# prj-beatrice/beatrice-vst

Measured on AMD Instinct MI355X. Metric: audio frames/sec (24 kHz out, 10 ms hop), higher is better.
Workload: dtype f32

## Files before the change

### beatrice-vst_amd/csrc/ring.h

```cpp
#pragma once
#include <hip/hip_runtime.h>

struct Ring {
  float* base;
  int C;
  int n;
  int m;
};

template <class T>
__device__ __forceinline__ T* as_global(T* p) {
  const unsigned long long v = reinterpret_cast<unsigned long long>(p);
  const unsigned long long u = (unsigned long long)(unsigned)__builtin_amdgcn_readfirstlane((int)(unsigned)v) |
                               ((unsigned long long)(unsigned)__builtin_amdgcn_readfirstlane((int)(unsigned)(v >> 32)) << 32);
  __attribute__((address_space(1))) T* g = (__attribute__((address_space(1))) T*)reinterpret_cast<T*>(u);
  asm("" : "+s"(g));
  return (T*)g;
}
template <class T>
__device__ __forceinline__ T* as_global_v(T* p) {
  __attribute__((address_space(1))) T* g = (__attribute__((address_space(1))) T*)p;
  asm("" : "+v"(g));
  return (T*)g;
}
__device__ __forceinline__ void globalize(Ring& r) { r.base = as_global(r.base); }

__host__ __device__ inline int ring_frames(const Ring& r) { return r.n * r.m; }
__host__ __device__ inline size_t ring_stream_floats(const Ring& r) { return (size_t)r.n * r.m * r.C; }

__device__ __forceinline__ int ring_pos(const Ring& r, int hop) { return (hop % r.m) * r.n; }

__device__ __forceinline__ float* ring_frame(const Ring& r, int b, int pos, int rel) {
  int f = pos + rel;
  const int R = r.n * r.m;
  if (f < 0) f += R;
  return r.base + (unsigned)(b * R + f) * (unsigned)r.C;
}

namespace stepc {
__shared__ int pair[2];
__shared__ const int* hopv;
constexpr unsigned long long kImmediateTop = 1ull << 36;
constexpr int kImmediateMaxSlot = 4095;
constexpr unsigned kImmediateHopMask = 0xffffffu;
__host__ __device__ inline const int* immediate(int hop, int slot = 0) {
  return reinterpret_cast<const int*>(static_cast<unsigned long long>((unsigned)(hop + 2)) | (static_cast<unsigned long long>((unsigned)slot) << 24));
}
__device__ __forceinline__ int step(const int* p) {
  const unsigned long long v = reinterpret_cast<unsigned long long>(p);
  return v == 0 ? pair[0] : (v < kImmediateTop ? (int)((unsigned)v & kImmediateHopMask) - 2 : *p);
}
__device__ __forceinline__ int of(const int* p, const int hop, const int b) {
  if (reinterpret_cast<unsigned long long>(p) != 0) return hop;
  const int* v = hopv;
  return v != nullptr ? v[b] : hop;
}
__device__ __forceinline__ bool ragged(const int* p) { return reinterpret_cast<unsigned long long>(p) == 0 && hopv != nullptr; }
template <bool RAG> __device__ __forceinline__ int of_t(const int hop, const int b) {
  if constexpr (RAG) { const int* v = hopv; return v != nullptr ? v[b] : hop; }
  else return hop;
}
template <bool RAG> __device__ __forceinline__ bool rag_t() {
  if constexpr (RAG) return hopv != nullptr;
  else return false;
}
__device__ __forceinline__ int slot(const int* p) {
  const unsigned long long v = reinterpret_cast<unsigned long long>(p);
  return v == 0 ? pair[1] : (v < kImmediateTop ? (int)(v >> 24) : p[1]);
}
template <class A> __device__ __forceinline__ auto set_hop(A& a, const int* p, int) -> decltype((void)(a.hop = p)) { a.hop = p; }
template <class A> __device__ __forceinline__ auto set_hop(A& a, const int* p, long) -> decltype((void)(a.a.hop = p)) { a.a.hop = p; }
template <class A> __device__ __forceinline__ void set_hop(A&, const int*, ...) {}
}
```

### beatrice-vst_amd/csrc/rowchain.hip.h

```cpp
#pragma once
#include "meas_env.h"
#include <hip/hip_runtime.h>

#include <cstdlib>

#include "conv_gemm.hip.h"
#include "kernels_misc.hip.h"
#include "ring.h"
#include "spec_math.hip.h"

#ifdef ABL_WEIGHTS_HOT
#define ABL_KB(x) ((x) & 1)
#else
#define ABL_KB(x) (x)
#endif

#ifdef RC_TIMING
__device__ unsigned long long* g_rc_stamps;
#define RC_STAMP(i) do { if (threadIdx.x == 0) g_rc_stamps[(size_t)blockIdx.x * 16 + (i)] = __builtin_readcyclecounter(); } while (0)
#else
#define RC_STAMP(i) do { } while (0)
#endif

namespace rc {

constexpr int NTHR = 512, NWAVE = 8;
#ifndef RC_KPERM
#define RC_KPERM 1
#endif
constexpr bool KPERM = RC_KPERM != 0;
constexpr int AS = B_HID + (KPERM ? 8 : 2);
constexpr int TILE = 16 * AS;
constexpr int SS = B_KV_LEN + (KPERM ? 8 : 2);
constexpr int STILE = 16 * SS;
__host__ __device__ constexpr int kpos(int k) { return KPERM ? ((k & ~15) | ((k & 3) << 2) | ((k >> 2) & 3)) : k; }
constexpr int KSTEP = KPERM ? 4 : 1;
#ifndef RC_WMAP
#define RC_WMAP RC_KPERM
#endif
template <int ROWGROUPS >
__device__ __forceinline__ void piece_of(const int W, const int ln, int* r, int* q) {
  if constexpr (RC_WMAP != 0) { *r = 4 * (W % ROWGROUPS) + (ln >> 4); *q = 16 * (W / ROWGROUPS) + (ln & 15); }
  else { *r = W; *q = ln; }
}
__device__ __forceinline__ int lane_koff(const int lane) { return KPERM ? 4 * (lane >> 4) : (lane >> 4); }
__device__ __forceinline__ float4 lds_kblock(const float* __restrict__ p, const int kb) {
  if constexpr (KPERM) return *reinterpret_cast<const float4*>(p + kb * 16);
  else { const float* q = p + kb * 16; return make_float4(q[0], q[4], q[8], q[12]); }
}
__device__ __forceinline__ void store_perm4(float* __restrict__ row, const int n0, const float v0, const float v1, const float v2, const float v3) {
  if constexpr (KPERM) {
    float* d = row + kpos(n0);
    d[0] = v0; d[4] = v1; d[8] = v2; d[12] = v3;
  } else {
    float2* d = reinterpret_cast<float2*>(row + n0);
    d[0] = make_float2(v0, v1); d[1] = make_float2(v2, v3);
  }
}

#ifndef RC_PIN_PIPELINE
#define RC_PIN_PIPELINE 1
#endif
__device__ __forceinline__ void pin_pipeline() {
#if RC_PIN_PIPELINE
  asm volatile("" ::: "memory");
  __builtin_amdgcn_sched_barrier(0);
#endif
}
#ifndef RC_PREFETCH
#define RC_PREFETCH 8
#endif
template <int RT, int CG> __host__ __device__ constexpr int seg_depth() { return RT == 1 ? (CG <= 2 ? RC_PREFETCH : (CG <= 3 ? 4 : 2)) : (RT * CG <= 2 ? 8 : 4); }
template <int RT, int CG> struct SegHead { float4 v[seg_depth<RT, CG>()][CG]; };
template <int RT, int CG>
__device__ __forceinline__ void seg_head_load(SegHead<RT, CG>& h, const float4* const (&wf)[CG]) {
#pragma unroll
  for (int d = 0; d < seg_depth<RT, CG>(); ++d)
#pragma unroll
    for (int c = 0; c < CG; ++c) h.v[d][c] = wf[c][(size_t)d * 64];
}
template <int CG, int KB, bool HEAD = false>
__device__ __forceinline__ void mma_segment_p(f32x4 (&acc)[CG], const float* __restrict__ a, const float4* const (&wf)[CG], const SegHead<1, CG>* head = nullptr) {
  constexpr int D = seg_depth<1, CG>();
  static_assert(KB % D == 0, "segment length");
  float4 bq[D][CG];
  pin_pipeline();
#pragma unroll
  for (int d = 0; d < D; ++d)
#pragma unroll
    for (int c = 0; c < CG; ++c) { if constexpr (HEAD) bq[d][c] = head->v[d][c]; else bq[d][c] = wf[c][(size_t)d * 64]; }
  float4 an = lds_kblock(a, 0);
#pragma unroll
  for (int kb = 0; kb < KB; kb += D) {
#pragma unroll
    for (int d = 0; d < D; ++d) {
      float4 cur[CG];
#pragma unroll
      for (int c = 0; c < CG; ++c) cur[c] = bq[d][c];
      const float4 x = an;
      if (kb + d + D < KB) {
#pragma unroll
        for (int c = 0; c < CG; ++c) bq[d][c] = wf[c][(size_t)ABL_KB(kb + d + D) * 64];
      }
      if (kb + d + 1 < KB) an = lds_kblock(a, kb + d + 1);
      pin_pipeline();
#pragma unroll
      for (int c = 0; c < CG; ++c) acc[c] = __builtin_amdgcn_mfma_f32_16x16x4f32(cur[c].x, x.x, acc[c], 0, 0, 0);
#pragma unroll
      for (int c = 0; c < CG; ++c) acc[c] = __builtin_amdgcn_mfma_f32_16x16x4f32(cur[c].y, x.y, acc[c], 0, 0, 0);
#pragma unroll
      for (int c = 0; c < CG; ++c) acc[c] = __builtin_amdgcn_mfma_f32_16x16x4f32(cur[c].z, x.z, acc[c], 0, 0, 0);
#pragma unroll
      for (int c = 0; c < CG; ++c) acc[c] = __builtin_amdgcn_mfma_f32_16x16x4f32(cur[c].w, x.w, acc[c], 0, 0, 0);
    }
  }
}
template <int RT, int CG, int KB, bool HEAD = false>
__device__ __forceinline__ void mma_segment_rt(f32x4 (&acc)[RT][CG], const float* __restrict__ a, const int a_tile_stride,
                                               const float4* const (&wf)[CG], const SegHead<RT, CG>* head = nullptr) {
  constexpr int D = seg_depth<RT, CG>();
  static_assert(KB % D == 0, "segment length");
  float4 bq[D][CG];
  pin_pipeline();
#pragma unroll
  for (int d = 0; d < D; ++d)
#pragma unroll
    for (int c = 0; c < CG; ++c) { if constexpr (HEAD) bq[d][c] = head->v[d][c]; else bq[d][c] = wf[c][(size_t)d * 64]; }
  float4 an[RT];
#pragma unroll
  for (int t = 0; t < RT; ++t) an[t] = lds_kblock(a + t * a_tile_stride, 0);
#pragma unroll
  for (int kb = 0; kb < KB; kb += D) {
#pragma unroll
    for (int d = 0; d < D; ++d) {
      float4 cur[CG];
#pragma unroll
      for (int c = 0; c < CG; ++c) cur[c] = bq[d][c];
      float4 av[RT];
#pragma unroll
      for (int t = 0; t < RT; ++t) av[t] = an[t];
      if (kb + d + D < KB) {
#pragma unroll
        for (int c = 0; c < CG; ++c) bq[d][c] = wf[c][(size_t)ABL_KB(kb + d + D) * 64];
      }
      if (kb + d + 1 < KB) {
#pragma unroll
        for (int t = 0; t < RT; ++t) an[t] = lds_kblock(a + t * a_tile_stride, kb + d + 1);
      }
      pin_pipeline();
#pragma unroll
      for (int t = 0; t < RT; ++t)
#pragma unroll
        for (int c = 0; c < CG; ++c) acc[t][c] = __builtin_amdgcn_mfma_f32_16x16x4f32(cur[c].x, av[t].x, acc[t][c], 0, 0, 0);
#pragma unroll
      for (int t = 0; t < RT; ++t)
#pragma unroll
        for (int c = 0; c < CG; ++c) acc[t][c] = __builtin_amdgcn_mfma_f32_16x16x4f32(cur[c].y, av[t].y, acc[t][c], 0, 0, 0);
#pragma unroll
      for (int t = 0; t < RT; ++t)
#pragma unroll
        for (int c = 0; c < CG; ++c) acc[t][c] = __builtin_amdgcn_mfma_f32_16x16x4f32(cur[c].z, av[t].z, acc[t][c], 0, 0, 0);
#pragma unroll
      for (int t = 0; t < RT; ++t)
#pragma unroll
        for (int c = 0; c < CG; ++c) acc[t][c] = __builtin_amdgcn_mfma_f32_16x16x4f32(cur[c].w, av[t].w, acc[t][c], 0, 0, 0);
    }
  }
}
template <int CG, int KB>
__device__ __forceinline__ void mma_segment(f32x4 (&acc)[CG], const float* __restrict__ a, const float4* __restrict__ wf,
                                            const size_t tile_stride) {
  const float4* wfc[CG];
#pragma unroll
  for (int c = 0; c < CG; ++c) wfc[c] = wf + c * tile_stride;
  mma_segment_p<CG, KB>(acc, a, wfc);
}

template <int NSEG, int CG, class Epi4>
__device__ __forceinline__ void layer256(const float* const (&seg)[NSEG], const int as, const float* __restrict__ w_packed,
                                         const int wave, const int lane, Epi4 epi4) {
  constexpr int K = NSEG * 256;
  const float4* wf = reinterpret_cast<const float4*>(w_packed) + (size_t)wave * (K / 16) * 64 + lane;
  const size_t tile_stride = (size_t)NWAVE * (K / 16) * 64;
  f32x4 tot[CG];
#pragma unroll
  for (int s = 0; s < NSEG; ++s) {
    f32x4 acc[CG];
#pragma unroll
    for (int c = 0; c < CG; ++c) acc[c] = f32x4{0.f, 0.f, 0.f, 0.f};
    mma_segment<CG, 16>(acc, seg[s] + (lane & 15) * as + lane_koff(lane), wf + (size_t)s * 16 * 64, tile_stride);
#pragma unroll
    for (int c = 0; c < CG; ++c) {
      if (s == 0) tot[c] = acc[c];
      else { tot[c][0] = tot[c][0] + acc[c][0]; tot[c][1] = tot[c][1] + acc[c][1]; tot[c][2] = tot[c][2] + acc[c][2]; tot[c][3] = tot[c][3] + acc[c][3]; }
    }
  }
#pragma unroll
  for (int c = 0; c < CG; ++c) epi4(lane & 15, (wave + NWAVE * c) * 16 + (lane >> 4) * 4, tot[c]);
}

template <int HOPS = 1>
__device__ __forceinline__ void load_tile(float* __restrict__ dst, const Ring& ring, const int* sid , const int pos, const int rel,
                                          const int tid, const int* rowhop = nullptr) {
#pragma unroll
  for (int i = 0; i < 2; ++i) {
    const int idx = tid + i * NTHR;
    int r, q;
    piece_of<4>(idx >> 6, idx & 63, &r, &q);
    const int b = sid[r];
    float4 v = make_float4(0.f, 0.f, 0.f, 0.f);
    if (b >= 0) v = *reinterpret_cast<const float4*>(ring_frame(ring, b / HOPS, rowhop != nullptr ? ring_pos(ring, rowhop[r]) : pos, rel + b % HOPS) + 4 * q);
    store_perm4(dst + r * AS, 4 * q, v.x, v.y, v.z, v.w);
  }
}

struct BlockAArgs {
  Ring x, xa;
  const float *c1_w, *c1_b, *c2_w, *c2_b;
  const int* hop;
  int B;
};
__device__ __forceinline__ void globalize(BlockAArgs& a) {
  globalize(a.x); globalize(a.xa);
  a.c1_w = as_global(a.c1_w); a.c1_b = as_global(a.c1_b); a.c2_w = as_global(a.c2_w); a.c2_b = as_global(a.c2_b); a.hop = as_global(a.hop);
}
constexpr int kBlockALds = 4 * TILE + 32;
template <int D, bool RAG = false, int HOPS = 1>
__device__ __forceinline__ void block_a_body(const BlockAArgs& a, const int g, float* __restrict__ lds) {
  float* T[3] = {lds, lds + TILE, lds + 2 * TILE};
  float* Hh = lds + 3 * TILE;
  int* sid = reinterpret_cast<int*>(lds + 4 * TILE);
  int* rowhop_ = sid + 16;
  const int tid = threadIdx.x, lane = tid & 63, wave = tid >> 6;
  const int hop = stepc::step(a.hop);
  if (hop < 0) return;
  const int* rowhop = stepc::rag_t<RAG>() ? rowhop_ : nullptr;
  if (tid < 16) {
    const int b = g * 16 + tid < a.B * HOPS ? g * 16 + tid : -1;
    const int hr = b >= 0 ? stepc::of_t<RAG>(hop, b / HOPS) : -1;
    sid[tid] = hr >= 0 ? b : -1;
    rowhop_[tid] = hr >= 0 ? hr : 0;
  }
  __syncthreads();
  const int pos = ring_pos(a.x, hop);
#pragma unroll
  for (int j = 0; j < 3; ++j) load_tile<HOPS>(T[j], a.x, sid, pos, -(2 - j) * D, tid, rowhop);
  __syncthreads();
  {
    const float* const seg[3] = {T[0], T[1], T[2]};
    const float* __restrict__ bias = a.c1_b;
    layer256<3, 2>(seg, AS, a.c1_w, wave, lane, [&](int r, int n0, const f32x4& v) {
      const float4 bn = *reinterpret_cast<const float4*>(bias + n0);
      const bsp::f32x2 g0 = bsp::gelu2(bsp::f32x2{v[0] + bn.x, v[1] + bn.y}), g1 = bsp::gelu2(bsp::f32x2{v[2] + bn.z, v[3] + bn.w});
      store_perm4(Hh + r * AS, n0, g0.x, g0.y, g1.x, g1.y);
    });
  }
  __syncthreads();
  {
    const float* const seg[1] = {Hh};
    const float* __restrict__ bias = a.c2_b;
    const int pos_o = ring_pos(a.xa, hop);
    layer256<1, 2>(seg, AS, a.c2_w, wave, lane, [&](int r, int n0, const f32x4& v) {
      const int b = sid[r];
      if (b < 0) return;
      const float4 bn = *reinterpret_cast<const float4*>(bias + n0);
      const float* x = T[2] + r * AS + kpos(n0);
      *reinterpret_cast<float4*>(ring_frame(a.xa, b / HOPS, rowhop != nullptr ? ring_pos(a.xa, rowhop[r]) : pos_o, b % HOPS) + n0) =
          make_float4(x[0] + (v[0] + bn.x), x[KSTEP] + (v[1] + bn.y), x[2 * KSTEP] + (v[2] + bn.z), x[3 * KSTEP] + (v[3] + bn.w));
    });
  }
}
template <int D, int HOPS = 1>
struct BlockAOp {
  using Args = BlockAArgs;
  static constexpr int NTHR = rc::NTHR;
  static constexpr int LDS_FLOATS = kBlockALds;
  static inline dim3 grid(const Args& a) { return dim3((a.B * HOPS + 15) / 16, 1); }
  static inline bhip::LaunchInfo info(const Args& a) {
    return bhip::LaunchInfo{"wave.blk.a", 2.0 * a.B * HOPS * (768.0 + 256.0) * 256.0, 4.0 * ((768.0 + 256.0) * 256.0 + a.B * HOPS * 5.0 * 256.0)};
  }
  static constexpr double wg_cost() { return 20.0; }
  __device__ static __forceinline__ void run(const Args& a, int bx, int, float* lds) { block_a_body<D, false, HOPS>(a, bx, lds); }
  template <bool RAG> __device__ static __forceinline__ void run_t(const Args& a, int bx, int, float* lds) { block_a_body<D, RAG, HOPS>(a, bx, lds); }
};
template <int D>
static __global__ __launch_bounds__(NTHR, 4) void block_a_kernel(const BlockAArgs a) {
  __shared__ __attribute__((aligned(16))) float lds[kBlockALds];
  block_a_body<D>(a, blockIdx.x, lds);
}

struct BlockBArgs {
  Ring xa, out;
  const float *q_w, *q_b, *o_w, *o_b;
  const float *kt, *v;
  const int* perm;
  const int* tile_slot;
  const int* hop;
};
__device__ __forceinline__ void globalize(BlockBArgs& a) {
  globalize(a.xa); globalize(a.out);
  a.q_w = as_global(a.q_w); a.q_b = as_global(a.q_b); a.o_w = as_global(a.o_w); a.o_b = as_global(a.o_b);
  a.kt = as_global(a.kt); a.v = as_global(a.v); a.perm = as_global(a.perm); a.tile_slot = as_global(a.tile_slot); a.hop = as_global(a.hop);
}
constexpr int kBlockBLds = 2 * TILE + STILE + 48;
template <bool RAG = false, int HOPS = 1>
__device__ __forceinline__ void block_b_body(const BlockBArgs& a, const int g, float* __restrict__ lds) {
  float* XA = lds;
  float* Q = lds + TILE;
  float* S = lds + 2 * TILE;
  float* inv = S + STILE;
  int* sid = reinterpret_cast<int*>(inv + 16);
  const int tid = threadIdx.x, lane = tid & 63, wave = tid >> 6;
  const int hop = stepc::step(a.hop);
  if (hop < 0) return;
  const int slot = a.tile_slot[g];
  if (slot < 0) return;
  RC_STAMP(0);
  int* rowhop_ = sid + 16;
  const int* rowhop = stepc::rag_t<RAG>() ? rowhop_ : nullptr;
  if (tid < 16) {
    const int b = a.perm[g * 16 + tid];
    const int hr = b >= 0 ? stepc::of_t<RAG>(hop, b / HOPS) : -1;
    sid[tid] = hr >= 0 ? b : -1;
    rowhop_[tid] = hr >= 0 ? hr : 0;
  }
  __syncthreads();
  load_tile<HOPS>(XA, a.xa, sid, ring_pos(a.xa, hop), 0, tid, rowhop);
  __syncthreads();
  {
    const float* const seg[1] = {XA};
    const float* __restrict__ bias = a.q_b;
    RC_STAMP(1);
    layer256<1, 2>(seg, AS, a.q_w, wave, lane, [&](int r, int n0, const f32x4& v) {
      const float4 bn = *reinterpret_cast<const float4*>(bias + n0);
      store_perm4(Q + r * AS, n0, v[0] + bn.x, v[1] + bn.y, v[2] + bn.z, v[3] + bn.w);
    });
  }
  __syncthreads();
  RC_STAMP(2);
  {
    const float* const seg[1] = {Q};
    layer256<1, 3>(seg, AS, a.kt + (size_t)slot * B_HID * B_KV_LEN, wave, lane, [&](int r, int n0, const f32x4& v) {
      store_perm4(S + r * SS, n0, v[0] * 0.0625f, v[1] * 0.0625f, v[2] * 0.0625f, v[3] * 0.0625f);
    });
  }
  __syncthreads();
  RC_STAMP(3);
  const int lp = kpos(lane);
#pragma unroll
  for (int rr = 0; rr < 2; ++rr) {
    const int r = wave * 2 + rr;
    float v[6];
#pragma unroll
    for (int i = 0; i < 6; ++i) v[i] = S[r * SS + lp + 64 * i];
    float mx = -__builtin_huge_valf();
#pragma unroll
    for (int i = 0; i < 6; ++i) mx = fmaxf(mx, v[i]);
    mx = bsp::wmax64(mx);
    float s = 0.0f;
#pragma unroll
    for (int i = 0; i < 6; i += 2) {
      const bsp::f32x2 e = bsp::exp2(bsp::f32x2{v[i] - mx, v[i + 1] - mx});
      s = s + e.x; s = s + e.y;
      S[r * SS + lp + 64 * i] = e.x; S[r * SS + lp + 64 * (i + 1)] = e.y;
    }
    const float tot = bsp::wsum64(s);
    if (lane == 0) inv[r] = 1.0f / tot;
  }
  __syncthreads();
  RC_STAMP(4);
  {
    const float4* wf = reinterpret_cast<const float4*>(a.v + (size_t)slot * B_KV_LEN * B_HID) + (size_t)wave * (B_KV_LEN / 16) * 64 + lane;
    const size_t tile_stride = (size_t)NWAVE * (B_KV_LEN / 16) * 64;
    const float* ap = S + (lane & 15) * SS + lane_koff(lane);
    f32x4 acc0[2] = {f32x4{0.f, 0.f, 0.f, 0.f}, f32x4{0.f, 0.f, 0.f, 0.f}}, acc1[2] = {f32x4{0.f, 0.f, 0.f, 0.f}, f32x4{0.f, 0.f, 0.f, 0.f}};
    mma_segment<2, 16>(acc0, ap, wf, tile_stride);
    mma_segment<2, 8>(acc1, ap + 256, wf + (size_t)16 * 64, tile_stride);
    const int r = lane & 15;
    const float ir = inv[r];
#pragma unroll
    for (int c = 0; c < 2; ++c)
      store_perm4(Q + r * AS, (wave + NWAVE * c) * 16 + (lane >> 4) * 4, (acc0[c][0] + acc1[c][0]) * ir, (acc0[c][1] + acc1[c][1]) * ir,
                  (acc0[c][2] + acc1[c][2]) * ir, (acc0[c][3] + acc1[c][3]) * ir);
  }
  __syncthreads();
  RC_STAMP(5);
  {
    const float* const seg[1] = {Q};
    const float* __restrict__ bias = a.o_b;
    const int pos_o = ring_pos(a.out, hop);
    layer256<1, 2>(seg, AS, a.o_w, wave, lane, [&](int r, int n0, const f32x4& v) {
      const int b = sid[r];
      if (b < 0) return;
      const float4 bn = *reinterpret_cast<const float4*>(bias + n0);
      const float* x = XA + r * AS + kpos(n0);
      *reinterpret_cast<float4*>(ring_frame(a.out, b / HOPS, rowhop != nullptr ? ring_pos(a.out, rowhop[r]) : pos_o, b % HOPS) + n0) =
          make_float4(x[0] + (v[0] + bn.x), x[KSTEP] + (v[1] + bn.y), x[2 * KSTEP] + (v[2] + bn.z), x[3 * KSTEP] + (v[3] + bn.w));
    });
  }
  RC_STAMP(6);
}
template <int HOPS = 1>
struct BlockBOpH {
  using Args = BlockBArgs;
  static constexpr int NTHR = rc::NTHR;
  static constexpr int LDS_FLOATS = kBlockBLds;
  static constexpr double wg_cost() { return 24.0; }
  __device__ static __forceinline__ void run(const Args& a, int bx, int, float* lds) { block_b_body<false, HOPS>(a, bx, lds); }
  template <bool RAG> __device__ static __forceinline__ void run_t(const Args& a, int bx, int, float* lds) { block_b_body<RAG, HOPS>(a, bx, lds); }
};
using BlockBOp = BlockBOpH<1>;
static __global__ __launch_bounds__(NTHR, 4) void block_b_kernel(const BlockBArgs a) {
  __shared__ __attribute__((aligned(16))) float lds[kBlockBLds];
  block_b_body(a, blockIdx.x, lds);
}

template <int NV> struct QuadVec;
template <> struct QuadVec<1> { using T = float; };
template <> struct QuadVec<2> { using T = float2; };
template <> struct QuadVec<4> { using T = float4; };
__device__ __forceinline__ float quad_elem(const float4& v, int c) { return c == 0 ? v.x : c == 1 ? v.y : c == 2 ? v.z : v.w; }
__device__ __forceinline__ float quad_elem(const float2& v, int c) { return c == 0 ? v.x : v.y; }
__device__ __forceinline__ float quad_elem(const float& v, int) { return v; }
template <int NV, int KLEN, int LDB>
__device__ __forceinline__ void quad_segment(f32x4 (&acc)[NV], const float* __restrict__ a, const float* __restrict__ bp) {
  using V = typename QuadVec<NV>::T;
  constexpr int D = NV == 1 ? 32 : 64 / NV;
  constexpr int G = 8;
  static_assert(KLEN % D == 0 && D % G == 0, "segment length");
  V bq[D];
  float2 an[G / 2];
  pin_pipeline();
#pragma unroll
  for (int d = 0; d < D; ++d) bq[d] = *reinterpret_cast<const V*>(bp + (size_t)d * LDB);
#pragma unroll
  for (int d = 0; d < G / 2; ++d) an[d] = *reinterpret_cast<const float2*>(a + 2 * d);
#pragma unroll 1
  for (int k = 0; k < KLEN; k += D) {
    const bool more = k + D < KLEN;
#pragma unroll
    for (int g = 0; g < D; g += G) {
      float2 ac[G / 2];
#pragma unroll
      for (int d = 0; d < G / 2; ++d) ac[d] = an[d];
      if (k + g + G < KLEN) {
#pragma unroll
        for (int d = 0; d < G / 2; ++d) an[d] = *reinterpret_cast<const float2*>(a + k + g + G + 2 * d);
      }
      V cur[G];
#pragma unroll
      for (int d = 0; d < G; ++d) cur[d] = bq[g + d];
      if (more) {
#pragma unroll
        for (int d = 0; d < G; ++d) bq[g + d] = *reinterpret_cast<const V*>(bp + (size_t)(k + g + d + D) * LDB);
      }
      pin_pipeline();
#pragma unroll
      for (int d = 0; d < G; ++d)
#pragma unroll
        for (int c = 0; c < NV; ++c)
          acc[c] = __builtin_amdgcn_mfma_f32_4x4x1f32((d & 1) ? ac[d / 2].y : ac[d / 2].x, quad_elem(cur[d], c), acc[c], 0, 0, 0);
    }
  }
}
struct BlockBqArgs {
  Ring xa, out;
  const float *q_w, *q_b, *o_w, *o_b;
  const float *ktp, *vp;
  const int* qperm;
  const int* qslot;
  const int* hop;
};
__device__ __forceinline__ void globalize(BlockBqArgs& a) {
  globalize(a.xa); globalize(a.out);
  a.q_w = as_global(a.q_w); a.q_b = as_global(a.q_b); a.o_w = as_global(a.o_w); a.o_b = as_global(a.o_b);
  a.ktp = as_global(a.ktp); a.vp = as_global(a.vp); a.qperm = as_global(a.qperm); a.qslot = as_global(a.qslot); a.hop = as_global(a.hop);
}
constexpr int kBlockBqLds = kBlockBLds;
template <bool RAG = false, int HOPS = 1>
__device__ __forceinline__ void block_bq_body(const BlockBqArgs& a, const int g, float* __restrict__ lds) {
  float* XA = lds;
  float* Q = lds + TILE;
  float* S = lds + 2 * TILE;
  float* inv = S + STILE;
  int* sid = reinterpret_cast<int*>(inv + 16);
  const int tid = threadIdx.x, lane = tid & 63, wave = tid >> 6;
  const int wave_u = __builtin_amdgcn_readfirstlane(wave);
  const int hop = stepc::step(a.hop);
  if (hop < 0) return;
  const int2 qs = *reinterpret_cast<const int2*>(a.qslot + 2 * g);
  if (qs.x < 0 && qs.y < 0) return;
  __builtin_amdgcn_s_setprio(3);
  RC_STAMP(0);
  int* rowhop_ = sid + 16;
  const int* rowhop = stepc::rag_t<RAG>() ? rowhop_ : nullptr;
  if (tid < 16) {
    const int b = tid < 8 ? a.qperm[g * 8 + tid] : -1;
    const int hr = b >= 0 ? stepc::of_t<RAG>(hop, b / HOPS) : -1;
    sid[tid] = hr >= 0 ? b : -1;
    rowhop_[tid] = hr >= 0 ? hr : 0;
  }
  __syncthreads();
  load_tile<HOPS>(XA, a.xa, sid, ring_pos(a.xa, hop), 0, tid, rowhop);
  __syncthreads();
  {
    const float* const seg[1] = {XA};
    const float* __restrict__ bias = a.q_b;
    RC_STAMP(1);
    layer256<1, 2>(seg, AS, a.q_w, wave, lane, [&](int r, int n0, const f32x4& v) {
      const float4 bn = *reinterpret_cast<const float4*>(bias + n0);
      float2* d = reinterpret_cast<float2*>(Q + r * AS + n0);
      d[0] = make_float2(v[0] + bn.x, v[1] + bn.y); d[1] = make_float2(v[2] + bn.z, v[3] + bn.w);
    });
  }
  __syncthreads();
  RC_STAMP(2);
  const int quad = wave_u >> 2, part = wave_u & 3;
  const int my_slot = quad == 0 ? qs.x : qs.y;
  const int arow = quad * 4 + (lane & 3);
  if (part < 3) {
    f32x4 acc[2] = {f32x4{0.f, 0.f, 0.f, 0.f}, f32x4{0.f, 0.f, 0.f, 0.f}};
    const int j = part * 128 + 2 * lane;
    if (my_slot >= 0) quad_segment<2, B_HID, B_KV_LEN>(acc, Q + arow * AS, a.ktp + (size_t)my_slot * B_HID * B_KV_LEN + j);
#pragma unroll
    for (int r = 0; r < 4; ++r)
#pragma unroll
      for (int c = 0; c < 2; ++c) S[(quad * 4 + r) * SS + j + c] = acc[c][r] * 0.0625f;
  }
  __syncthreads();
  RC_STAMP(3);
  {
    const int r = wave;
    float v[6];
#pragma unroll
    for (int i = 0; i < 6; ++i) v[i] = S[r * SS + lane + 64 * i];
    float mx = -__builtin_huge_valf();
#pragma unroll
    for (int i = 0; i < 6; ++i) mx = fmaxf(mx, v[i]);
    mx = bsp::wmax64(mx);
    float s = 0.0f;
#pragma unroll
    for (int i = 0; i < 6; i += 2) {
      const bsp::f32x2 e = bsp::exp2(bsp::f32x2{v[i] - mx, v[i + 1] - mx});
      s = s + e.x; s = s + e.y;
      S[r * SS + lane + 64 * i] = e.x; S[r * SS + lane + 64 * (i + 1)] = e.y;
    }
    const float tot = bsp::wsum64(s);
    if (lane == 0) inv[r] = 1.0f / tot;
  }
  __syncthreads();
  RC_STAMP(4);
  {
    const int n = part * 64 + lane;
    f32x4 acc0[1] = {f32x4{0.f, 0.f, 0.f, 0.f}}, acc1[1] = {f32x4{0.f, 0.f, 0.f, 0.f}};
    if (my_slot >= 0) {
      const float* vp = a.vp + (size_t)my_slot * B_KV_LEN * B_HID + n;
      quad_segment<1, 256, B_HID>(acc0, S + arow * SS, vp);
      quad_segment<1, 128, B_HID>(acc1, S + arow * SS + 256, vp + (size_t)256 * B_HID);
    }
#pragma unroll
    for (int r = 0; r < 4; ++r) {
      const float v = acc0[0][r] + acc1[0][r];
      Q[(quad * 4 + r) * AS + kpos(n)] = v * inv[quad * 4 + r];
    }
  }
  __syncthreads();
  RC_STAMP(5);
  {
    const float* const seg[1] = {Q};
    const float* __restrict__ bias = a.o_b;
    const int pos_o = ring_pos(a.out, hop);
    layer256<1, 2>(seg, AS, a.o_w, wave, lane, [&](int r, int n0, const f32x4& v) {
      const int b = sid[r];
      if (b < 0) return;
      const float4 bn = *reinterpret_cast<const float4*>(bias + n0);
      const float* x = XA + r * AS + kpos(n0);
      *reinterpret_cast<float4*>(ring_frame(a.out, b / HOPS, rowhop != nullptr ? ring_pos(a.out, rowhop[r]) : pos_o, b % HOPS) + n0) =
          make_float4(x[0] + (v[0] + bn.x), x[KSTEP] + (v[1] + bn.y), x[2 * KSTEP] + (v[2] + bn.z), x[3 * KSTEP] + (v[3] + bn.w));
    });
  }
  __builtin_amdgcn_s_setprio(0);
  RC_STAMP(6);
}
template <int HOPS = 1>
struct BlockBqOpH {
  using Args = BlockBqArgs;
  static constexpr int NTHR = rc::NTHR;
  static constexpr int LDS_FLOATS = kBlockBqLds;
  static constexpr double wg_cost() { return 30.0; }
  __device__ static __forceinline__ void run(const Args& a, int bx, int, float* lds) { block_bq_body<false, HOPS>(a, bx, lds); }
  template <bool RAG> __device__ static __forceinline__ void run_t(const Args& a, int bx, int, float* lds) { block_bq_body<RAG, HOPS>(a, bx, lds); }
};
using BlockBqOp = BlockBqOpH<1>;
constexpr int kConvRowsLds = 2 * TILE + 32;
template <int RT> constexpr int conv_rows_lds() { return 2 * RT * TILE + 48 * RT; }
template <class L, int COLS = 0, int RT = 1, bool RAG = false>
__device__ __forceinline__ void conv_rows_body(const ConvArgs& a, const int bx, const int by, float* __restrict__ lds) {
  constexpr int NCOL = COLS > 0 ? COLS : L::NOUT;
  static_assert(L::NOUT % NCOL == 0 && NCOL % 16 == 0, "column slabs");
  constexpr int K = L::K, P = L::P, NTL = NCOL / 16, CG = (NTL + NWAVE - 1) / NWAVE;
  constexpr int ROWS = 16 * RT;
  const int nt_base = by * NTL;
  constexpr int LAST = K - 256 * (P - 1);
  static_assert(K % 16 == 0 && LAST % 64 == 0 && L::NOUT % 16 == 0 && !L::GROUPED, "layer shape");
  float* slot[2] = {lds, lds + RT * TILE};
  int* rb_ = reinterpret_cast<int*>(lds + 2 * RT * TILE);
  const int tid = threadIdx.x, lane = tid & 63, wave = tid >> 6;
  const int hop = stepc::step(a.hop);
  if (hop < 0) return;
  const float4* wfc[CG];
#pragma unroll
  for (int c = 0; c < CG; ++c) {
    const int nt = wave + NWAVE * c < NTL ? wave + NWAVE * c : NTL - 1;
    wfc[c] = reinterpret_cast<const float4*>(a.w) + (size_t)(nt_base + nt) * (K / 16) * 64 + lane;
  }
#ifndef RC_SEG_HEAD
#define RC_SEG_HEAD 0
#endif
  SegHead<RT, CG> head;
  if constexpr (RC_SEG_HEAD != 0) seg_head_load<RT, CG>(head, wfc);
  const int M = a.B * L::T;
  const bool rag = stepc::rag_t<RAG>();
  if (tid < ROWS) {
    const int m = bx * ROWS + tid;
    const int b = m < M ? m / L::T : -1;
    const int hr = b >= 0 ? stepc::of_t<RAG>(hop, b) : -1;
    rb_[tid] = hr >= 0 ? b : -1;
    rb_[ROWS + tid] = m < M ? m % L::T : 0;
    rb_[2 * ROWS + tid] = hr >= 0 ? hr : 0;
  }
  __syncthreads();
  const int pos_in = ring_pos(a.in, hop);
  int pr[2 * RT], pq[2 * RT], pb[2 * RT], pt[2 * RT];
#pragma unroll
  for (int i = 0; i < 2 * RT; ++i) {
    piece_of<4 * RT>(wave + NWAVE * i, lane, &pr[i], &pq[i]);
    pb[i] = rb_[pr[i]]; pt[i] = rb_[ROWS + pr[i]];
  }
  float4 nx[2 * RT];
  auto load_seg = [&](int s) {
#pragma unroll
    for (int i = 0; i < 2 * RT; ++i) {
      const int kk = s * 256 + 4 * pq[i];
      const bool live = kk < K;
      const int j = live ? kk / L::CIN : 0, c = live ? kk % L::CIN : 0;
      nx[i] = make_float4(0.f, 0.f, 0.f, 0.f);
      if (live && pb[i] >= 0)
        nx[i] = *reinterpret_cast<const float4*>(ring_frame(a.in, pb[i], rag ? ring_pos(a.in, rb_[2 * ROWS + pr[i]]) : pos_in,
                                                            (pt[i] + 1) * L::STRIDE - 1 - (L::KSZ - 1 - j) * L::DIL + a.rel_shift) + c);
    }
  };
  auto store_seg = [&](float* dst) {
#pragma unroll
    for (int i = 0; i < 2 * RT; ++i) {
      float4 v = nx[i];
      if constexpr (L::PRE == PRE_LRELU) { v.x = bsp::lrelu(v.x); v.y = bsp::lrelu(v.y); v.z = bsp::lrelu(v.z); v.w = bsp::lrelu(v.w); }
      store_perm4(dst + pr[i] * AS, 4 * pq[i], v.x, v.y, v.z, v.w);
    }
  };
  load_seg(0);
  store_seg(slot[0]);
  __syncthreads();
  f32x4 tot[RT][CG];
#pragma unroll
  for (int s = 0; s < P; ++s) {
    if (s + 1 < P) load_seg(s + 1);
    f32x4 acc[RT][CG];
#pragma unroll
    for (int t = 0; t < RT; ++t)
#pragma unroll
      for (int c = 0; c < CG; ++c) acc[t][c] = f32x4{0.f, 0.f, 0.f, 0.f};
    const float4* wfs[CG];
#pragma unroll
    for (int c = 0; c < CG; ++c) wfs[c] = wfc[c] + (size_t)s * 16 * 64;
    const float* ap = slot[s & 1] + (lane & 15) * AS + lane_koff(lane);
    if (RC_SEG_HEAD != 0 && s == 0) {
      if constexpr (RT == 1) {
        if constexpr (P > 1) mma_segment_p<CG, 16, true>(acc[0], ap, wfs, &head);
        else mma_segment_p<CG, LAST / 16, true>(acc[0], ap, wfs, &head);
      } else {
        if constexpr (P > 1) mma_segment_rt<RT, CG, 16, true>(acc, ap, TILE, wfs, &head);
        else mma_segment_rt<RT, CG, LAST / 16, true>(acc, ap, TILE, wfs, &head);
      }
    } else if constexpr (RT == 1) {
      if (s + 1 < P) mma_segment_p<CG, 16>(acc[0], ap, wfs);
      else mma_segment_p<CG, LAST / 16>(acc[0], ap, wfs);
    } else {
      if (s + 1 < P) mma_segment_rt<RT, CG, 16>(acc, ap, TILE, wfs);
      else mma_segment_rt<RT, CG, LAST / 16>(acc, ap, TILE, wfs);
    }
#pragma unroll
    for (int t = 0; t < RT; ++t)
#pragma unroll
      for (int c = 0; c < CG; ++c) {
        if (s == 0) tot[t][c] = acc[t][c];
        else { tot[t][c][0] = tot[t][c][0] + acc[t][c][0]; tot[t][c][1] = tot[t][c][1] + acc[t][c][1]; tot[t][c][2] = tot[t][c][2] + acc[t][c][2]; tot[t][c][3] = tot[t][c][3] + acc[t][c][3]; }
      }
    if (s + 1 < P) {
      store_seg(slot[(s + 1) & 1]);
      __syncthreads();
    }
  }
  const int pos_out = ring_pos(a.out, hop), R_out = a.out.n * a.out.m;
  int pos_res = 0, R_res = 0;
  if constexpr (L::RES) { pos_res = ring_pos(a.res, hop); R_res = a.res.n * a.res.m; }
  float4 bias_n[CG];
#pragma unroll
  for (int c = 0; c < CG; ++c) {
    const int nt = wave + NWAVE * c < NTL ? wave + NWAVE * c : NTL - 1;
    bias_n[c] = L::EPI == EPI_BIAS ? *reinterpret_cast<const float4*>(a.bias + (nt_base + nt) * 16 + (lane >> 4) * 4) : make_float4(0.f, 0.f, 0.f, 0.f);
  }
#pragma unroll
  for (int t = 0; t < RT; ++t) {
    const int r = 16 * t + (lane & 15);
    const int rb = rb_[r], rf = rb_[ROWS + r];
    int po = pos_out, pr = pos_res;
    if (rag) {
      const int hr = rb_[2 * ROWS + r];
      po = ring_pos(a.out, hr);
      if constexpr (L::RES) pr = ring_pos(a.res, hr);
    }
    float rs = 1.0f;
    if constexpr (L::EPI == EPI_ROWSCALE) rs = a.rowscale[(rb < 0 ? 0 : rb) * L::T + rf];
#pragma unroll
    for (int c = 0; c < CG; ++c) {
      if (wave + NWAVE * c >= NTL) continue;
      const int n0 = (nt_base + wave + NWAVE * c) * 16 + (lane >> 4) * 4;
      float v[4];
#pragma unroll
      for (int e = 0; e < 4; ++e) v[e] = tot[t][c][e];
      if constexpr (L::EPI == EPI_BIAS) { v[0] = v[0] + bias_n[c].x; v[1] = v[1] + bias_n[c].y; v[2] = v[2] + bias_n[c].z; v[3] = v[3] + bias_n[c].w; }
      if constexpr (L::EPI == EPI_SCALE) { for (int e = 0; e < 4; ++e) v[e] = v[e] * a.scale; }
      if constexpr (L::EPI == EPI_ROWSCALE) { for (int e = 0; e < 4; ++e) v[e] = v[e] * rs; }
      if constexpr (L::ACT == ACT_GELU) {
        const bsp::f32x2 g0 = bsp::gelu2(bsp::f32x2{v[0], v[1]}), g1 = bsp::gelu2(bsp::f32x2{v[2], v[3]});
        v[0] = g0.x; v[1] = g0.y; v[2] = g1.x; v[3] = g1.y;
      }
      if (rb < 0) continue;
      if constexpr (L::RES) {
        const float4 x = *reinterpret_cast<const float4*>(a.res.base + ((unsigned)(rb * R_res + pr) * (unsigned)a.res.C + (unsigned)(rf * L::NOUT + n0)));
        v[0] = x.x + v[0]; v[1] = x.y + v[1]; v[2] = x.z + v[2]; v[3] = x.w + v[3];
      }
      *reinterpret_cast<float4*>(a.out.base + ((unsigned)(rb * R_out + po) * (unsigned)a.out.C + (unsigned)(rf * L::NOUT + n0))) = make_float4(v[0], v[1], v[2], v[3]);
    }
  }
}
template <class L, int COLS = 0, int RT = 1>
struct ConvRowsOp {
  using Args = ConvArgs;
  static constexpr int NTHR = rc::NTHR;
  static constexpr int LDS_FLOATS = conv_rows_lds<RT>();
  static inline dim3 grid(const ConvArgs& a) { return dim3((a.B * L::T + 16 * RT - 1) / (16 * RT), COLS > 0 ? L::NOUT / COLS : 1); }
  static inline bhip::LaunchInfo info(const char* name, const ConvArgs& a) { return ConvOp<L, TileCfg<1, 1, 1, 2, 1>>::info(name, a); }
  __device__ static __forceinline__ void run(const ConvArgs& a, int bx, int by, float* lds) { conv_rows_body<L, COLS, RT>(a, bx, by, lds); }
  template <bool RAG> __device__ static __forceinline__ void run_t(const ConvArgs& a, int bx, int by, float* lds) { conv_rows_body<L, COLS, RT, RAG>(a, bx, by, lds); }
};

struct NopOp {
  struct Args { int unused; };
  static constexpr int NTHR = 64;
  static constexpr int LDS_FLOATS = 0;
  __device__ static __forceinline__ void run(const Args&, int, int, float*) {}
  template <bool RAG> __device__ static __forceinline__ void run_t(const Args&, int, int, float*) {}
};
__device__ __forceinline__ void globalize(NopOp::Args&) {}

template <class L, int COLS, int RT>
static __global__ __launch_bounds__(NTHR, 4) void conv_rows_kernel(const ConvArgs a) {
  __shared__ __attribute__((aligned(16))) float lds[conv_rows_lds<RT>()];
  conv_rows_body<L, COLS, RT>(a, blockIdx.x, blockIdx.y, lds);
}
template <class L, int COLS = 0, int RT = 2>
static inline void launch_conv_rows(const char* name, const ConvArgs& a, hipStream_t stream) {
  using Op = ConvRowsOp<L, COLS, RT>;
  bhip::launch_site(Op::info(name, a), stream, [&] { hipLaunchKernelGGL((conv_rows_kernel<L, COLS, RT>), Op::grid(a), dim3(NTHR), 0, stream, a); });
}

}

template <class L>
static inline void launch_many_rows(const char* name, const ConvArgs& a, hipStream_t s) {
  constexpr int LAST = L::K - 256 * (L::P - 1);
  constexpr bool ok = !L::GROUPED && L::K % 16 == 0 && LAST % 64 == 0 && L::NOUT % 16 == 0;
  if constexpr (ok) {
    static const bool off = bhip::meas_env("BEATRICE_HIP_NO_CONVROWS") != nullptr;
    if (!off) {
      constexpr int COLS = (L::NOUT % 128 == 0 && (L::NOUT > 256 || (L::NOUT == 256 && L::K >= 768))) ? 128 : 0;
      rc::launch_conv_rows<L, COLS, 2>(name, a, s);
      return;
    }
  }
  launch_conv<L, TL>(name, a, 0, s);
}
```

Measured before the change: 4.349 million.

## Stream weights via global-address-space SGPR base with VGPR offsets and defer gather

Introduces a WStream abstraction that addresses packed weights through an SGPR-held global-address-space base plus a per-lane byte offset and immediate offsets, instead of per-lane 64-bit flat pointers. Ring reads in load_tile and the conv gather also use a scalar global base plus a 32-bit index. The next segment's activation gather now runs inside the MMA segment, after the first weight prefetches are issued, rather than before them. The aim is fewer VGPRs and address instructions, global rather than flat loads, and earlier weight loads that overlap the gather. This relies on inline-asm address-space tricks and offset arithmetic that must stay correct for every kb.

```diff
diff --git a/beatrice-vst_amd/csrc/ring.h b/beatrice-vst_amd/csrc/ring.h
--- a/beatrice-vst_amd/csrc/ring.h
+++ b/beatrice-vst_amd/csrc/ring.h
@@ -30,12 +30,13 @@
 
 __device__ __forceinline__ int ring_pos(const Ring& r, int hop) { return (hop % r.m) * r.n; }
 
-__device__ __forceinline__ float* ring_frame(const Ring& r, int b, int pos, int rel) {
+__device__ __forceinline__ unsigned ring_index(const Ring& r, int b, int pos, int rel) {
   int f = pos + rel;
   const int R = r.n * r.m;
   if (f < 0) f += R;
-  return r.base + (unsigned)(b * R + f) * (unsigned)r.C;
+  return (unsigned)(b * R + f) * (unsigned)r.C;
 }
+__device__ __forceinline__ float* ring_frame(const Ring& r, int b, int pos, int rel) { return r.base + ring_index(r, b, pos, rel); }
 
 namespace stepc {
 __shared__ int pair[2];
diff --git a/beatrice-vst_amd/csrc/rowchain.hip.h b/beatrice-vst_amd/csrc/rowchain.hip.h
--- a/beatrice-vst_amd/csrc/rowchain.hip.h
+++ b/beatrice-vst_amd/csrc/rowchain.hip.h
@@ -70,25 +70,57 @@
 #ifndef RC_PREFETCH
 #define RC_PREFETCH 8
 #endif
+#ifndef RC_WSTREAM_GLOBAL
+#define RC_WSTREAM_GLOBAL 1
+#endif
+struct WLane {
+  const float4* p;
+  __device__ static __forceinline__ WLane make(const float4* u, const int lane) { return WLane{u + lane}; }
+  __device__ __forceinline__ WLane at(const size_t f4) const { return WLane{p + f4}; }
+  __device__ __forceinline__ float4 kblock(const int kb) const { return p[(size_t)kb * 64]; }
+};
+struct WGlobal {
+  typedef __attribute__((address_space(1))) const char gbyte;
+  gbyte* base;
+  unsigned voff;
+  __device__ static __forceinline__ WGlobal make(const float4* u, const int lane) {
+    return WGlobal{(gbyte*)reinterpret_cast<const char*>(as_global(u)), (unsigned)lane * 16u};
+  }
+  __device__ __forceinline__ WGlobal at(const size_t f4) const { return WGlobal{base + f4 * 16, voff}; }
+  __device__ __forceinline__ float4 kblock(const int kb) const {
+    gbyte* q = base + ((size_t)(kb & ~7) * 1024 + 4096);
+    asm("" : "+s"(q));
+    const f32x4 v = *reinterpret_cast<__attribute__((address_space(1))) const f32x4*>(q + (size_t)voff + ((kb & 7) * 1024 - 4096));
+    return make_float4(v[0], v[1], v[2], v[3]);
+  }
+};
+#if RC_WSTREAM_GLOBAL
+using WStream = WGlobal;
+#else
+using WStream = WLane;
+#endif
+struct NoGather { __device__ __forceinline__ void operator()() const {} };
 template <int RT, int CG> __host__ __device__ constexpr int seg_depth() { return RT == 1 ? (CG <= 2 ? RC_PREFETCH : (CG <= 3 ? 4 : 2)) : (RT * CG <= 2 ? 8 : 4); }
 template <int RT, int CG> struct SegHead { float4 v[seg_depth<RT, CG>()][CG]; };
-template <int RT, int CG>
-__device__ __forceinline__ void seg_head_load(SegHead<RT, CG>& h, const float4* const (&wf)[CG]) {
+template <int RT, int CG, class W>
+__device__ __forceinline__ void seg_head_load(SegHead<RT, CG>& h, const W (&wf)[CG]) {
 #pragma unroll
   for (int d = 0; d < seg_depth<RT, CG>(); ++d)
 #pragma unroll
-    for (int c = 0; c < CG; ++c) h.v[d][c] = wf[c][(size_t)d * 64];
-}
-template <int CG, int KB, bool HEAD = false>
-__device__ __forceinline__ void mma_segment_p(f32x4 (&acc)[CG], const float* __restrict__ a, const float4* const (&wf)[CG], const SegHead<1, CG>* head = nullptr) {
-  constexpr int D = seg_depth<1, CG>();
+    for (int c = 0; c < CG; ++c) h.v[d][c] = wf[c].kblock(d);
+}
+template <int CG, int KB, bool HEAD = false, int D = seg_depth<1, CG>(), class W, class Gather = NoGather>
+__device__ __forceinline__ void mma_segment_p(f32x4 (&acc)[CG], const float* __restrict__ a, const W (&wf)[CG], const SegHead<1, CG>* head = nullptr,
+                                              Gather gather = Gather()) {
   static_assert(KB % D == 0, "segment length");
+  static_assert(!HEAD || D == seg_depth<1, CG>(), "a SegHead holds seg_depth() k-blocks");
   float4 bq[D][CG];
   pin_pipeline();
 #pragma unroll
   for (int d = 0; d < D; ++d)
 #pragma unroll
-    for (int c = 0; c < CG; ++c) { if constexpr (HEAD) bq[d][c] = head->v[d][c]; else bq[d][c] = wf[c][(size_t)d * 64]; }
+    for (int c = 0; c < CG; ++c) { if constexpr (HEAD) bq[d][c] = head->v[d][c]; else bq[d][c] = wf[c].kblock(d); }
+  gather();
   float4 an = lds_kblock(a, 0);
 #pragma unroll
   for (int kb = 0; kb < KB; kb += D) {
@@ -100,7 +132,7 @@
       const float4 x = an;
       if (kb + d + D < KB) {
 #pragma unroll
-        for (int c = 0; c < CG; ++c) bq[d][c] = wf[c][(size_t)ABL_KB(kb + d + D) * 64];
+        for (int c = 0; c < CG; ++c) bq[d][c] = wf[c].kblock(ABL_KB(kb + d + D));
       }
       if (kb + d + 1 < KB) an = lds_kblock(a, kb + d + 1);
       pin_pipeline();
@@ -115,17 +147,18 @@
     }
   }
 }
-template <int RT, int CG, int KB, bool HEAD = false>
+template <int RT, int CG, int KB, bool HEAD = false, int D = seg_depth<RT, CG>(), class W, class Gather = NoGather>
 __device__ __forceinline__ void mma_segment_rt(f32x4 (&acc)[RT][CG], const float* __restrict__ a, const int a_tile_stride,
-                                               const float4* const (&wf)[CG], const SegHead<RT, CG>* head = nullptr) {
-  constexpr int D = seg_depth<RT, CG>();
+                                               const W (&wf)[CG], const SegHead<RT, CG>* head = nullptr, Gather gather = Gather()) {
   static_assert(KB % D == 0, "segment length");
+  static_assert(!HEAD || D == seg_depth<RT, CG>(), "a SegHead holds seg_depth() k-blocks");
   float4 bq[D][CG];
   pin_pipeline();
 #pragma unroll
   for (int d = 0; d < D; ++d)
 #pragma unroll
-    for (int c = 0; c < CG; ++c) { if constexpr (HEAD) bq[d][c] = head->v[d][c]; else bq[d][c] = wf[c][(size_t)d * 64]; }
+    for (int c = 0; c < CG; ++c) { if constexpr (HEAD) bq[d][c] = head->v[d][c]; else bq[d][c] = wf[c].kblock(d); }
+  gather();
   float4 an[RT];
 #pragma unroll
   for (int t = 0; t < RT; ++t) an[t] = lds_kblock(a + t * a_tile_stride, 0);
@@ -141,7 +174,7 @@
       for (int t = 0; t < RT; ++t) av[t] = an[t];
       if (kb + d + D < KB) {
 #pragma unroll
-        for (int c = 0; c < CG; ++c) bq[d][c] = wf[c][(size_t)ABL_KB(kb + d + D) * 64];
+        for (int c = 0; c < CG; ++c) bq[d][c] = wf[c].kblock(ABL_KB(kb + d + D));
       }
       if (kb + d + 1 < KB) {
 #pragma unroll
@@ -167,12 +200,11 @@
     }
   }
 }
-template <int CG, int KB>
-__device__ __forceinline__ void mma_segment(f32x4 (&acc)[CG], const float* __restrict__ a, const float4* __restrict__ wf,
-                                            const size_t tile_stride) {
-  const float4* wfc[CG];
-#pragma unroll
-  for (int c = 0; c < CG; ++c) wfc[c] = wf + c * tile_stride;
+template <int CG, int KB, class W>
+__device__ __forceinline__ void mma_segment(f32x4 (&acc)[CG], const float* __restrict__ a, const W& wf, const size_t tile_stride) {
+  W wfc[CG];
+#pragma unroll
+  for (int c = 0; c < CG; ++c) wfc[c] = wf.at(c * tile_stride);
   mma_segment_p<CG, KB>(acc, a, wfc);
 }
 
@@ -180,7 +212,7 @@
 __device__ __forceinline__ void layer256(const float* const (&seg)[NSEG], const int as, const float* __restrict__ w_packed,
                                          const int wave, const int lane, Epi4 epi4) {
   constexpr int K = NSEG * 256;
-  const float4* wf = reinterpret_cast<const float4*>(w_packed) + (size_t)wave * (K / 16) * 64 + lane;
+  const WStream wf = WStream::make(reinterpret_cast<const float4*>(w_packed) + (size_t)wave * (K / 16) * 64, lane);
   const size_t tile_stride = (size_t)NWAVE * (K / 16) * 64;
   f32x4 tot[CG];
 #pragma unroll
@@ -188,7 +220,7 @@
     f32x4 acc[CG];
 #pragma unroll
     for (int c = 0; c < CG; ++c) acc[c] = f32x4{0.f, 0.f, 0.f, 0.f};
-    mma_segment<CG, 16>(acc, seg[s] + (lane & 15) * as + lane_koff(lane), wf + (size_t)s * 16 * 64, tile_stride);
+    mma_segment<CG, 16>(acc, seg[s] + (lane & 15) * as + lane_koff(lane), wf.at((size_t)s * 16 * 64), tile_stride);
 #pragma unroll
     for (int c = 0; c < CG; ++c) {
       if (s == 0) tot[c] = acc[c];
@@ -202,6 +234,7 @@
 template <int HOPS = 1>
 __device__ __forceinline__ void load_tile(float* __restrict__ dst, const Ring& ring, const int* sid , const int pos, const int rel,
                                           const int tid, const int* rowhop = nullptr) {
+  const float* gbase = as_global(ring.base);
 #pragma unroll
   for (int i = 0; i < 2; ++i) {
     const int idx = tid + i * NTHR;
@@ -209,7 +242,7 @@
     piece_of<4>(idx >> 6, idx & 63, &r, &q);
     const int b = sid[r];
     float4 v = make_float4(0.f, 0.f, 0.f, 0.f);
-    if (b >= 0) v = *reinterpret_cast<const float4*>(ring_frame(ring, b / HOPS, rowhop != nullptr ? ring_pos(ring, rowhop[r]) : pos, rel + b % HOPS) + 4 * q);
+    if (b >= 0) v = *reinterpret_cast<const float4*>(gbase + (ring_index(ring, b / HOPS, rowhop != nullptr ? ring_pos(ring, rowhop[r]) : pos, rel + b % HOPS) + 4u * (unsigned)q));
     store_perm4(dst + r * AS, 4 * q, v.x, v.y, v.z, v.w);
   }
 }
@@ -370,12 +403,12 @@
   __syncthreads();
   RC_STAMP(4);
   {
-    const float4* wf = reinterpret_cast<const float4*>(a.v + (size_t)slot * B_KV_LEN * B_HID) + (size_t)wave * (B_KV_LEN / 16) * 64 + lane;
+    const WStream wf = WStream::make(reinterpret_cast<const float4*>(a.v + (size_t)slot * B_KV_LEN * B_HID) + (size_t)wave * (B_KV_LEN / 16) * 64, lane);
     const size_t tile_stride = (size_t)NWAVE * (B_KV_LEN / 16) * 64;
     const float* ap = S + (lane & 15) * SS + lane_koff(lane);
     f32x4 acc0[2] = {f32x4{0.f, 0.f, 0.f, 0.f}, f32x4{0.f, 0.f, 0.f, 0.f}}, acc1[2] = {f32x4{0.f, 0.f, 0.f, 0.f}, f32x4{0.f, 0.f, 0.f, 0.f}};
     mma_segment<2, 16>(acc0, ap, wf, tile_stride);
-    mma_segment<2, 8>(acc1, ap + 256, wf + (size_t)16 * 64, tile_stride);
+    mma_segment<2, 8>(acc1, ap + 256, wf.at((size_t)16 * 64), tile_stride);
     const int r = lane & 15;
     const float ir = inv[r];
 #pragma unroll
@@ -608,11 +641,11 @@
   const int tid = threadIdx.x, lane = tid & 63, wave = tid >> 6;
   const int hop = stepc::step(a.hop);
   if (hop < 0) return;
-  const float4* wfc[CG];
+  WStream wfc[CG];
 #pragma unroll
   for (int c = 0; c < CG; ++c) {
     const int nt = wave + NWAVE * c < NTL ? wave + NWAVE * c : NTL - 1;
-    wfc[c] = reinterpret_cast<const float4*>(a.w) + (size_t)(nt_base + nt) * (K / 16) * 64 + lane;
+    wfc[c] = WStream::make(reinterpret_cast<const float4*>(a.w) + (size_t)(nt_base + nt) * (K / 16) * 64, lane);
   }
 #ifndef RC_SEG_HEAD
 #define RC_SEG_HEAD 0
@@ -638,6 +671,7 @@
     pb[i] = rb_[pr[i]]; pt[i] = rb_[ROWS + pr[i]];
   }
   float4 nx[2 * RT];
+  const float* in_base = as_global(a.in.base);
   auto load_seg = [&](int s) {
 #pragma unroll
     for (int i = 0; i < 2 * RT; ++i) {
@@ -646,8 +680,8 @@
       const int j = live ? kk / L::CIN : 0, c = live ? kk % L::CIN : 0;
       nx[i] = make_float4(0.f, 0.f, 0.f, 0.f);
       if (live && pb[i] >= 0)
-        nx[i] = *reinterpret_cast<const float4*>(ring_frame(a.in, pb[i], rag ? ring_pos(a.in, rb_[2 * ROWS + pr[i]]) : pos_in,
-                                                            (pt[i] + 1) * L::STRIDE - 1 - (L::KSZ - 1 - j) * L::DIL + a.rel_shift) + c);
+        nx[i] = *reinterpret_cast<const float4*>(in_base + (ring_index(a.in, pb[i], rag ? ring_pos(a.in, rb_[2 * ROWS + pr[i]]) : pos_in,
+                                                                       (pt[i] + 1) * L::STRIDE - 1 - (L::KSZ - 1 - j) * L::DIL + a.rel_shift) + (unsigned)c));
     }
   };
   auto store_seg = [&](float* dst) {
@@ -664,30 +698,30 @@
   f32x4 tot[RT][CG];
 #pragma unroll
   for (int s = 0; s < P; ++s) {
-    if (s + 1 < P) load_seg(s + 1);
+    auto gather = [&] { if (s + 1 < P) load_seg(s + 1); };
     f32x4 acc[RT][CG];
 #pragma unroll
     for (int t = 0; t < RT; ++t)
 #pragma unroll
       for (int c = 0; c < CG; ++c) acc[t][c] = f32x4{0.f, 0.f, 0.f, 0.f};
-    const float4* wfs[CG];
-#pragma unroll
-    for (int c = 0; c < CG; ++c) wfs[c] = wfc[c] + (size_t)s * 16 * 64;
+    WStream wfs[CG];
+#pragma unroll
+    for (int c = 0; c < CG; ++c) wfs[c] = wfc[c].at((size_t)s * 16 * 64);
     const float* ap = slot[s & 1] + (lane & 15) * AS + lane_koff(lane);
     if (RC_SEG_HEAD != 0 && s == 0) {
       if constexpr (RT == 1) {
-        if constexpr (P > 1) mma_segment_p<CG, 16, true>(acc[0], ap, wfs, &head);
-        else mma_segment_p<CG, LAST / 16, true>(acc[0], ap, wfs, &head);
+        if constexpr (P > 1) mma_segment_p<CG, 16, true>(acc[0], ap, wfs, &head, gather);
+        else mma_segment_p<CG, LAST / 16, true>(acc[0], ap, wfs, &head, gather);
       } else {
-        if constexpr (P > 1) mma_segment_rt<RT, CG, 16, true>(acc, ap, TILE, wfs, &head);
-        else mma_segment_rt<RT, CG, LAST / 16, true>(acc, ap, TILE, wfs, &head);
+        if constexpr (P > 1) mma_segment_rt<RT, CG, 16, true>(acc, ap, TILE, wfs, &head, gather);
+        else mma_segment_rt<RT, CG, LAST / 16, true>(acc, ap, TILE, wfs, &head, gather);
       }
     } else if constexpr (RT == 1) {
-      if (s + 1 < P) mma_segment_p<CG, 16>(acc[0], ap, wfs);
-      else mma_segment_p<CG, LAST / 16>(acc[0], ap, wfs);
+      if (s + 1 < P) mma_segment_p<CG, 16>(acc[0], ap, wfs, nullptr, gather);
+      else mma_segment_p<CG, LAST / 16>(acc[0], ap, wfs, nullptr, gather);
     } else {
-      if (s + 1 < P) mma_segment_rt<RT, CG, 16>(acc, ap, TILE, wfs);
-      else mma_segment_rt<RT, CG, LAST / 16>(acc, ap, TILE, wfs);
+      if (s + 1 < P) mma_segment_rt<RT, CG, 16>(acc, ap, TILE, wfs, nullptr, gather);
+      else mma_segment_rt<RT, CG, LAST / 16>(acc, ap, TILE, wfs, nullptr, gather);
     }
 #pragma unroll
     for (int t = 0; t < RT; ++t)
```

Result: faster. 4.555 million, median of 6 (+4.7%).
